# Lagrange-Labs/mapreduce-plonky2

Measured on AMD Instinct MI355X. Metric: leaf proofs/sec (whole node) + NTT GB/s vs HBM peak, 2^20-row table build, 1/2/4/8 GPU, higher is better.
Workload: dtype u64 (Goldilocks field)

## Files before the change

### include/mp2g.h

```cpp
#ifndef MP2G_H
#define MP2G_H
#include <stddef.h>
#include <stdint.h>
#ifdef __cplusplus
extern "C" {
#endif

typedef struct mp2g_ctx mp2g_ctx;
typedef struct mp2g_tree mp2g_tree;
typedef struct mp2g_batch mp2g_batch;

#define MP2G_POSEIDON2 0
#define MP2G_POSEIDON 1

uint64_t mp2g_stat_leaf_permutations(void);
const char* mp2g_last_error(void);
int mp2g_device_count(void);
int mp2g_ctx_create(int device, mp2g_ctx** out);
void mp2g_ctx_destroy(mp2g_ctx* ctx);
int mp2g_ctx_sync(mp2g_ctx* ctx);
int mp2g_ctx_make_current(mp2g_ctx* ctx);
int mp2g_ctx_mem_info(mp2g_ctx* ctx, size_t* free_bytes, size_t* total_bytes);
void* mp2g_ctx_stream(mp2g_ctx* ctx);
int mp2g_ctx_set_stream(mp2g_ctx* ctx, void* stream);
// ... 238 lines not shown
enum mp2g_witness_op_wide {
  MP2G_OP_U32_INTERLEAVE = 48,
  MP2G_OP_UNINTERLEAVE_TO_B32 = 49,
  MP2G_OP_UNINTERLEAVE_TO_U32 = 50,
  MP2G_OP_U256_DIV = 51,
  MP2G_OP_BIGUINT_DIV_REM = 52,
  MP2G_OP_POSEIDON_MDS = 53,
  MP2G_OP_WIDE_END = 54
};
typedef struct mp2g_witness_program mp2g_witness_program;
int mp2g_witness_program_create(const uint64_t* tape, size_t tape_len, uint32_t n_slots, uint32_t log_n, const uint32_t* input_sids,
                                uint32_t n_inputs, const uint64_t* const_slots, uint32_t n_consts, mp2g_witness_program** out);
uint32_t mp2g_witness_program_num_inputs(const mp2g_witness_program* p);
int mp2g_witness_program_set_lookups(mp2g_witness_program* p, const mp2g_lookup* luts, uint32_t n_luts);
uint32_t mp2g_witness_program_num_levels(const mp2g_witness_program* p);
int mp2g_witness_program_set_probe(mp2g_witness_program* p, const uint32_t* probe_sids, uint32_t n_probe);
int mp2g_witness_program_run_dev(mp2g_witness_program* p, mp2g_ctx* ctx, const uint64_t* d_inputs, uint32_t batch, uint64_t* d_wires,
                                 uint64_t* d_probe_out);
int mp2g_witness_program_run(const mp2g_witness_program* p, const uint64_t* inputs, uint32_t batch, uint32_t threads, uint64_t* wires,
                             const uint32_t* probe_sids, uint32_t n_probe, uint64_t* probe_out);
int mp2g_witness_program_run_rows(const mp2g_witness_program* p, const uint64_t* inputs, uint32_t batch, uint32_t threads, uint64_t* rows,
                                  const uint32_t* probe_sids, uint32_t n_probe, uint64_t* probe_out);
int mp2g_wires_from_rows_dev(mp2g_ctx* ctx, const uint64_t* d_rows, uint64_t* d_wires, uint32_t log_n, uint32_t num_wires, uint32_t batch);
void mp2g_witness_program_free(mp2g_witness_program* p);

typedef struct mp2g_chain mp2g_chain;
typedef struct { uint32_t job; uint32_t offset; uint32_t n_words; uint32_t pad_; const uint64_t* d_src; } mp2g_chain_patch;
int mp2g_chain_create(mp2g_ctx* ctx, uint32_t n_steps, mp2g_prover* const* provers, mp2g_witness_program* const* programs,
                      const mp2g_fri_params* params, const uint64_t* const* d_circuit_digests, uint32_t capacity, mp2g_chain** out);
int mp2g_chain_run(mp2g_chain* chain, const uint64_t* inputs, uint32_t batch, const mp2g_chain_patch* patches, uint32_t n_patches,
                   uint64_t* caps, uint64_t* openings, uint64_t* proof, uint64_t* public_inputs);
int mp2g_chain_step_buffers(const mp2g_chain* chain, uint32_t step, uint64_t** d_wires, uint64_t** d_probe, uint64_t** d_caps,
                            uint64_t** d_openings, uint64_t** d_proof);
int mp2g_chain_device_proof(const mp2g_chain* chain, uint32_t b, const uint64_t* d_parts[4], uint32_t n_words[4]);
void mp2g_chain_free(mp2g_chain* chain);

typedef struct mp2g_forest mp2g_forest;
typedef struct {
  uint32_t n_inputs;
  uint32_t n_children;
  uint32_t child_offset[4];
  uint32_t n_const;
} mp2g_forest_circuit;
int mp2g_forest_create(uint32_t n_workers, mp2g_ctx* const* ctxs, uint32_t n_circuits, const mp2g_forest_circuit* circuits,
                       mp2g_chain* const* chains, uint32_t slot_words, uint32_t pool_slots, mp2g_forest** out);
int mp2g_forest_add_nodes(mp2g_forest* f, uint32_t circuit, uint32_t count, const uint64_t* ids, const uint64_t* child_ids ,
                          const uint64_t* consts , const uint8_t* keep );
int mp2g_forest_group_units(const uint32_t* item_sizes, uint32_t n_items, uint32_t n_workers, uint32_t group_nodes,
                            uint32_t* unit_first_item, uint32_t* n_units);
int mp2g_forest_prove(mp2g_forest* f, const uint64_t* unit_nodes, const uint32_t* unit_offsets , uint32_t n_units);
struct mp2g_update_plan;
int mp2g_forest_prove_plan(mp2g_forest* f, struct mp2g_update_plan* plan, uint32_t group_nodes, uint32_t n_satellites, uint32_t satellite_shift,
                           uint32_t* waves, uint32_t* items_per_wave, uint32_t max_waves);
int mp2g_forest_proof(mp2g_forest* f, uint64_t id, uint64_t* words, uint32_t* n_words);
int mp2g_forest_device_proof(mp2g_forest* f, uint64_t id, const uint64_t** d_words, uint32_t* n_words);
int mp2g_forest_release(mp2g_forest* f, uint64_t id);
int mp2g_forest_verify(mp2g_forest* f, mp2g_verifier* v, const uint64_t* ids, uint32_t n_ids, uint32_t* status);
uint64_t mp2g_forest_proved(const mp2g_forest* f);
uint32_t mp2g_forest_free_slots(mp2g_forest* f);
void mp2g_forest_free(mp2g_forest* f);

typedef struct mp2g_update_tree mp2g_update_tree;
typedef struct mp2g_update_plan mp2g_update_plan;
int mp2g_update_tree_from_paths(const uint64_t* keys, const uint32_t* path_lens, uint32_t n_paths, int64_t epoch,
                                mp2g_update_tree** out);
int mp2g_update_tree_from_map(const uint64_t* keys, const uint64_t* left, const uint64_t* right, const uint8_t* has_left,
                              const uint8_t* has_right, uint32_t n, uint64_t root, int64_t epoch, mp2g_update_tree** out);
int mp2g_update_tree_extend_with_path(mp2g_update_tree* t, const uint64_t* path, uint32_t len);
uint32_t mp2g_update_tree_size(const mp2g_update_tree* t);
int64_t mp2g_update_tree_epoch(const mp2g_update_tree* t);
int mp2g_update_tree_contains_key(const mp2g_update_tree* t, uint64_t k);
int mp2g_update_tree_nodes(const mp2g_update_tree* t, uint64_t* keys, int32_t* parents, uint8_t* is_path_end);
int mp2g_update_tree_subtree_size(const mp2g_update_tree* t, uint64_t k, uint32_t* out);
void mp2g_update_tree_free(mp2g_update_tree* t);
int mp2g_update_plan_create(mp2g_update_tree* t, uint32_t subtree_size, mp2g_update_plan** out);
#define MP2G_PLAN_FINISHED 0
#define MP2G_PLAN_READY 1
#define MP2G_PLAN_NOT_YET 2
int mp2g_update_plan_next(mp2g_update_plan* p, uint64_t* k, int* is_path_end, mp2g_update_tree** subtree);
int mp2g_update_plan_done(mp2g_update_plan* p, uint64_t k);
int mp2g_update_plan_completed(const mp2g_update_plan* p);
void mp2g_update_plan_free(mp2g_update_plan* p);

#ifdef __cplusplus
}
#endif
#endif
```

### mapreduce-plonky2_amd/__init__.py

```python
import ctypes
import time
import os
import weakref

import numpy as np

_HERE = os.path.dirname(os.path.abspath(__file__))
LIB_PATH = os.environ.get("MP2G_LIB", os.path.join(_HERE, "libmp2gpu.so"))
HEADER_PATH = os.path.join(os.path.dirname(_HERE), "include", "mp2g.h")

P = 0xFFFFFFFF00000001
MULT_GEN = 14293326489335486720
POSEIDON2, POSEIDON = 0, 1

_u64p = ctypes.POINTER(ctypes.c_uint64)
_u32p = ctypes.POINTER(ctypes.c_uint32)
_lib = None


class Mp2gError(RuntimeError):
    pass


def load():
# ... 658 lines not shown
    def free(self):
        if self.h and self.ctx.h:
            load().mp2g_chain_free(self.h)
        self.h = None

    def __del__(self):
        try:
            self.free()
        except Exception:
            pass


class ForestCircuit(ctypes.Structure):
    _fields_ = [("n_inputs", ctypes.c_uint32), ("n_children", ctypes.c_uint32), ("child_offset", ctypes.c_uint32 * 4), ("n_const", ctypes.c_uint32)]


class Forest:

    def __init__(self, ctxs, descriptors, chains, slot_words, pool_slots):
        self.ctxs, self.chains = list(ctxs), [list(row) for row in chains]
        nw, nc = len(ctxs), len(descriptors)
        d = (ForestCircuit * nc)()
        for i, (n_in, offs, n_const) in enumerate(descriptors):
            d[i].n_inputs, d[i].n_children, d[i].n_const = int(n_in), len(offs), int(n_const)
            for k, o in enumerate(offs):
                d[i].child_offset[k] = int(o)
        cx = (ctypes.c_void_p * nw)(*[c.h for c in ctxs])
        ch = (ctypes.c_void_p * (nw * nc))(*[(self.chains[w][c].h if self.chains[w][c] is not None else None) for w in range(nw) for c in range(nc)])
        self.h = ctypes.c_void_p()
        _ck(load().mp2g_forest_create(nw, cx, nc, d, ch, int(slot_words), int(pool_slots), ctypes.byref(self.h)))
        for c in self.ctxs:
            c._adopt(self)
        self.n_const = [int(x[2]) for x in descriptors]
        self.n_children = [len(x[1]) for x in descriptors]

    def add_nodes(self, circuit, ids, child_ids, consts, keep=None):
        ids = _arr(ids)
        n = ids.size
        kids = _arr(child_ids).reshape(n, self.n_children[circuit]) if self.n_children[circuit] else None
        cs = _arr(consts).reshape(n, self.n_const[circuit])
        kp = np.ascontiguousarray(keep, dtype=np.uint8) if keep is not None else None
        _ck(load().mp2g_forest_add_nodes(self.h, int(circuit), int(n), _p(ids), _p(kids) if kids is not None else None, _p(cs), _p(kp) if kp is not None else None))

    def prove(self, units):
        flat = _arr([i for u in units for i in u])
        offs = _arr(np.cumsum([0] + [len(u) for u in units]), np.uint32)
        _ck(load().mp2g_forest_prove(self.h, _p(flat), _p(offs), len(units)))

    def prove_plan(self, plan, group_nodes, n_satellites=0, satellite_shift=40):
        waves, per = ctypes.c_uint32(), (ctypes.c_uint32 * 64)()
        _ck(load().mp2g_forest_prove_plan(self.h, plan.h, int(group_nodes), int(n_satellites), int(satellite_shift), ctypes.byref(waves), per, 64))
        return [int(per[i]) for i in range(min(64, waves.value))]

    def proof_words(self, node_id):
        n = ctypes.c_uint32()
        _ck(load().mp2g_forest_proof(self.h, ctypes.c_uint64(int(node_id)), None, ctypes.byref(n)))
        out = np.empty(n.value, dtype=np.uint64)
        _ck(load().mp2g_forest_proof(self.h, ctypes.c_uint64(int(node_id)), _p(out), ctypes.byref(n)))
        return out

    def device_proof(self, node_id):
        ptr, n = ctypes.c_void_p(), ctypes.c_uint32()
        _ck(load().mp2g_forest_device_proof(self.h, ctypes.c_uint64(int(node_id)), ctypes.byref(ptr), ctypes.byref(n)))
        return int(ptr.value), int(n.value)

    def verify(self, ids, verifier):
        ids = _arr(ids)
        status = np.full(ids.size, 0xFFFFFFFF, dtype=np.uint32)
        _ck(load().mp2g_forest_verify(self.h, getattr(verifier, "v", verifier).h, _p(ids), int(ids.size), _p(status)))
        return status

    def release(self, node_id):
        _ck(load().mp2g_forest_release(self.h, ctypes.c_uint64(int(node_id))))

    @property
    def proved(self):
        load().mp2g_forest_proved.restype = ctypes.c_uint64
        return int(load().mp2g_forest_proved(self.h))

    def free(self):
        if self.h and all(c.h for c in self.ctxs):
            load().mp2g_forest_free(self.h)
        self.h = None

    def __del__(self):
        try:
            self.free()
        except Exception:
            pass


def map_to_curve_batch(ctx, inputs, variant=POSEIDON2, weierstrass=False):
    a = _arr(inputs)
    count, in_len = a.shape
    w = np.empty((count, 5), dtype=np.uint64)
    wei = np.empty((count, 11), dtype=np.uint64) if weierstrass else None
    _ck(load().mp2g_map_to_curve_batch(ctx.h, variant, _p(a), in_len, count, _p(w), _p(wei) if weierstrass else None))
    return (w, wei) if weierstrass else w


def swu_batch(ctx, u, weierstrass=False):
    a = _arr(u).reshape(-1, 5)
    count = a.shape[0]
    w = np.empty((count, 5), dtype=np.uint64)
    wei = np.empty((count, 11), dtype=np.uint64) if weierstrass else None
    _ck(load().mp2g_swu_batch(ctx.h, _p(a), count, _p(w), _p(wei) if weierstrass else None))
# ... 189 lines not shown
```

### mapreduce-plonky2_amd/csrc/forest.hip

```cpp
#include <algorithm>
#include <atomic>
#include <chrono>
#include <condition_variable>
#include <cstdlib>
#include <cstring>
#include <deque>
#include <exception>
#include <memory>
#include <mutex>
#include <new>
#include <string>
#include <thread>
#include <unordered_map>
#include <vector>
#include "chain.h"
#include "verifier.h"

using namespace mp2g;
extern "C" const char* mp2g_last_error(void);

namespace {
constexpr uint32_t MAX_CHILDREN = 4;
struct Node {
  uint64_t id = 0;
  uint32_t circuit = 0;
  uint32_t n_children = 0;
  uint64_t child[MAX_CHILDREN] = {0, 0, 0, 0};
  size_t consts = 0;
  int32_t slot = -1;
  uint32_t proof_words = 0;
  bool keep = false;
  bool proved = false;
  uint32_t queued_by = 0;
};
struct Circuit {
  mp2g_forest_circuit d{};
  std::vector<u64> consts;
};
struct Copy { const u64* src; u64* dst; uint32_t n; uint32_t pad; };
__global__ void __launch_bounds__(256) forest_copy_kernel(const Copy* jobs) {
  const Copy c = jobs[blockIdx.x];
  for (uint32_t i = threadIdx.x; i < c.n; i += 256) c.dst[i] = c.src[i];
}
}

struct mp2g_forest {
  uint32_t n_workers = 0, n_circuits = 0, slot_words = 0, pool_slots = 0;
  std::vector<mp2g_ctx*> ctxs;
  std::vector<mp2g_chain*> chains;
  std::vector<Circuit> circuits;
  std::unordered_map<uint64_t, uint32_t> index;
  std::vector<Node> nodes;
  DevBuf pool;
  std::vector<int32_t> free_slots;
  std::mutex mu;
  std::condition_variable slots_back;
  uint32_t active = 0, waiting = 0;
  std::atomic<uint64_t> proved{0};
  bool pipelined = true;
  static constexpr uint32_t RING = 3;
  struct Slot { Copy* h_jobs = nullptr; Copy* d_jobs = nullptr; uint32_t* h_flags = nullptr; hipEvent_t done = nullptr; };
  struct Worker { Slot ring[RING]; uint32_t cap_jobs = 0; uint32_t seq = 0; };
  std::vector<Worker> workers;
  ~mp2g_forest() {
    for (auto& w : workers)
      for (auto& r : w.ring) {
        if (r.h_jobs) (void)hipHostFree(r.h_jobs);
        if (r.d_jobs) (void)hipFree(r.d_jobs);
        if (r.h_flags) (void)hipHostFree(r.h_flags);
        if (r.done) (void)hipEventDestroy(r.done);
      }
  }
};

namespace {
struct BatchCtx {
  const Copy* d_jobs; uint32_t n_between, n_after;
};
int hook_copy(const Copy* d_jobs, uint32_t count, hipStream_t s) {
  if (!count) return 0;
  hipLaunchKernelGGL(forest_copy_kernel, dim3(count), dim3(256), 0, s, d_jobs);
  hipError_t e = hipGetLastError();
  return e == hipSuccess ? 0 : fail("forest copy kernel: %s", hipGetErrorString(e));
}
int hook_between(void* u, mp2g_chain*, hipStream_t s) { auto* b = (BatchCtx*)u; return hook_copy(b->d_jobs, b->n_between, s); }
int hook_after(void* u, mp2g_chain*, hipStream_t s) { auto* b = (BatchCtx*)u; return hook_copy(b->d_jobs + b->n_between, b->n_after, s); }

struct InFlight {
  uint32_t ring = 0, B = 0, out_words = 0;
  mp2g_chain* ch = nullptr;
  std::vector<uint32_t> nodes;
  std::vector<int32_t> slots;
};

int prove_unit_body(mp2g_forest* f, uint32_t w, const uint64_t* ids, uint32_t count, std::deque<InFlight>& flight);
int prove_unit(mp2g_forest* f, uint32_t w, const uint64_t* ids, uint32_t count) {
  std::deque<InFlight> flight;
  try {
    return prove_unit_body(f, w, ids, count, flight);
  } catch (...) {
    (void)hipStreamSynchronize(f->ctxs[w]->stream);
    {
      std::lock_guard<std::mutex> g(f->mu);
      for (InFlight& b : flight) {
        for (uint32_t i : b.nodes) { Node& n = f->nodes[i]; n.proved = false; n.queued_by = 0; n.slot = -1; n.proof_words = 0; }
        for (int32_t sl : b.slots) f->free_slots.push_back(sl);
      }
    }
    f->slots_back.notify_all();
    return fail("forest: out of memory (or another exception) inside a unit of worker %u: its queued batches were rolled back", w);
  }
}
// ... 136 lines not shown
            src += end - at;
            at = end;
            if (k < C.d.n_children) {
              Node* ch_node = nullptr;
              {
                std::lock_guard<std::mutex> g(f->mu);
                ch_node = &f->nodes[f->index[n.child[k]]];
                if (!(ch_node->proved || ch_node->queued_by == w + 1) || ch_node->slot < 0) return fail("forest: child %llu of node %llu is not proved (or was released)", (unsigned long long)n.child[k], (unsigned long long)n.id);
              }
              if (at + ch_node->proof_words > C.d.n_inputs) return fail("forest: circuit %u: a child proof runs past the inputs", c);
              R.h_jobs[nb++] = Copy{f->pool.p + (size_t)ch_node->slot * f->slot_words, s0.in.p + (size_t)j * s0.n_in + at, ch_node->proof_words, 0};
              at += ch_node->proof_words;
            }
          }
          if (at != C.d.n_inputs || src != C.consts.data() + n.consts + C.d.n_const)
            return fail("forest: circuit %u: the node's constant words and its children's proofs do not add up to the circuit's %u inputs", c, C.d.n_inputs);
        }
        return 0;
        }();
        if (arc) { give_back(); UNIT_FAIL(arc); }
        const uint32_t n_between = nb;
        for (uint32_t j = 0; j < B; j++) {
          u64* slot = f->pool.p + (size_t)slots[j] * f->slot_words;
          for (uint32_t k = 0; k < 4; k++) R.h_jobs[nb++] = Copy{L.part(k, j), slot + L.parts.off[k], L.parts.n[k], 0};
        }
        {
          hipError_t e = hipMemcpyAsync(R.d_jobs, R.h_jobs, (size_t)nb * sizeof(Copy), hipMemcpyHostToDevice, stream);
          if (e != hipSuccess) { give_back(); UNIT_FAIL(fail("forest: copy jobs upload: %s", hipGetErrorString(e))); }
        }
        memset(R.h_flags, 0, (size_t)ch->n_steps * ch->cap * sizeof(uint32_t));
        BatchCtx bc{R.d_jobs, n_between, nb - n_between};
        ChainHooks hooks{&bc, hook_between, hook_after};
        int rc = chain_enqueue(ch, B, which, &hooks, R.h_flags);
        if (!rc) { hipError_t e = hipEventRecord(R.done, stream); if (e != hipSuccess) rc = fail("forest: event record: %s", hipGetErrorString(e)); }
        if (rc) { std::string msg = mp2g_last_error(); (void)hipStreamSynchronize(stream); give_back(); roll_back(); return fail("%s", msg.c_str()); }
        InFlight fl;
        fl.ring = ring; fl.B = B; fl.out_words = out_words; fl.ch = ch; fl.slots = slots;
        fl.nodes.assign(todo.begin() + lo, todo.begin() + lo + B);
        {
          std::lock_guard<std::mutex> g(f->mu);
          for (uint32_t j = 0; j < B; j++) {
            Node& n = f->nodes[todo[lo + j]];
            n.slot = slots[j]; n.proof_words = out_words; n.queued_by = w + 1;
          }
        }
        flight.push_back(std::move(fl));
      }
    }
  }
  while (!flight.empty()) UNIT_FAIL(confirm_oldest());
#undef UNIT_FAIL
  return 0;
}
}


extern "C" {
int mp2g_forest_create(uint32_t n_workers, mp2g_ctx* const* ctxs, uint32_t n_circuits, const mp2g_forest_circuit* circuits,
                       mp2g_chain* const* chains, uint32_t slot_words, uint32_t pool_slots, mp2g_forest** out) {
  NEED(out && ctxs && circuits && chains && n_workers >= 1 && n_circuits >= 1 && slot_words >= 1 && pool_slots >= 1, "workers / circuits / chains / pool");
  try {
    std::unique_ptr<mp2g_forest> f(new mp2g_forest);
    f->n_workers = n_workers; f->n_circuits = n_circuits; f->slot_words = slot_words; f->pool_slots = pool_slots;
    f->ctxs.assign(ctxs, ctxs + n_workers);
    f->chains.assign(chains, chains + (size_t)n_workers * n_circuits);
    f->circuits.resize(n_circuits);
    uint32_t max_jobs = 0;
    for (uint32_t c = 0; c < n_circuits; c++) {
      const mp2g_forest_circuit& d = circuits[c];
      NEED(d.n_children <= MAX_CHILDREN && d.n_const <= d.n_inputs, "circuit descriptor");
      f->circuits[c].d = d;
      for (uint32_t w = 0; w < n_workers; w++) {
        mp2g_chain* ch = f->chains[(size_t)w * n_circuits + c];
        if (!ch) continue;
        NEED(ch->steps[0].n_in == d.n_inputs, "a chain's base circuit takes another number of inputs than its descriptor says");
        NEED(ch->ctx == ctxs[w], "a worker's chains live on the worker's context");
        max_jobs = std::max(max_jobs, ch->cap * (d.n_children + 4));
      }
    }
    for (uint32_t w = 0; w < n_workers; w++) NEED(ctxs[w] && ctxs[w]->device == ctxs[0]->device, "one forest = one GPU: every worker's context on the same device");
    CK(hipSetDevice(ctxs[0]->device));
    hipError_t e = f->pool.alloc((size_t)slot_words * pool_slots * sizeof(u64));
    if (e != hipSuccess) return fail("forest pool of %u x %u words: %s", pool_slots, slot_words, hipGetErrorString(e));
    f->free_slots.resize(pool_slots);
    for (uint32_t i = 0; i < pool_slots; i++) f->free_slots[i] = (int32_t)(pool_slots - 1 - i);
    f->workers.resize(n_workers);
    uint32_t max_flags = 1;
    for (mp2g_chain* ch : f->chains) if (ch) max_flags = std::max(max_flags, ch->n_steps * ch->cap);
    for (auto& w : f->workers) {
      w.cap_jobs = std::max(1u, max_jobs);
      for (auto& r : w.ring) {
        CK(hipHostMalloc((void**)&r.h_jobs, (size_t)w.cap_jobs * sizeof(Copy), hipHostMallocDefault));
        CK(hipMalloc((void**)&r.d_jobs, (size_t)w.cap_jobs * sizeof(Copy)));
        CK(hipHostMalloc((void**)&r.h_flags, (size_t)max_flags * sizeof(uint32_t), hipHostMallocDefault));
        CK(hipEventCreateWithFlags(&r.done, hipEventDisableTiming));
      }
    }
    { const char* e = getenv("MP2G_FOREST_SYNC"); f->pipelined = !(e && atoi(e)); }
    *out = f.release();
    return 0;
  } catch (const std::bad_alloc&) { return fail("out of memory"); } catch (...) { return fail("internal error"); }
}

int mp2g_forest_add_nodes(mp2g_forest* f, uint32_t circuit, uint32_t count, const uint64_t* ids, const uint64_t* child_ids, const uint64_t* consts,
                          const uint8_t* keep) {
  NEED(f && circuit < f->n_circuits && (ids || !count), "forest / circuit / ids");
  Circuit& C = f->circuits[circuit];
  NEED((child_ids || !C.d.n_children || !count) && (consts || !C.d.n_const || !count), "children / constant words");
  try {
    {
      std::unordered_map<uint64_t, uint32_t> seen;
      seen.reserve(count);
      for (uint32_t i = 0; i < count; i++)
        if (f->index.count(ids[i]) || !seen.emplace(ids[i], i).second) return fail("forest: node %llu registered twice", (unsigned long long)ids[i]);
    }
    for (uint32_t i = 0; i < count; i++) {
      Node n;
      n.id = ids[i]; n.circuit = circuit; n.n_children = C.d.n_children;
      for (uint32_t k = 0; k < C.d.n_children; k++) n.child[k] = child_ids[(size_t)i * C.d.n_children + k];
      n.consts = C.consts.size();
      n.keep = keep && keep[i];
      C.consts.insert(C.consts.end(), consts + (size_t)i * C.d.n_const, consts + (size_t)(i + 1) * C.d.n_const);
      f->index.emplace(n.id, (uint32_t)f->nodes.size());
      f->nodes.push_back(n);
    }
    return 0;
  } catch (const std::bad_alloc&) { return fail("out of memory"); } catch (...) { return fail("internal error"); }
}

int mp2g_forest_prove(mp2g_forest* f, const uint64_t* unit_nodes, const uint32_t* unit_offsets, uint32_t n_units) {
  NEED(f && (n_units == 0 || (unit_nodes && unit_offsets)), "forest / units");
  if (!n_units) return 0;
  std::atomic<uint32_t> next{0};
  std::atomic<int> failed{0};
  std::mutex err_mu;
  std::string err;
  auto leave = [&]() { { std::lock_guard<std::mutex> g(f->mu); if (f->active) f->active--; } f->slots_back.notify_all(); };
  auto work = [&](uint32_t w) {
    struct Leave { decltype(leave)& fn; ~Leave() { fn(); } } on_exit{leave};
    try {
      for (;;) {
        if (failed.load()) return;
        const uint32_t u = next.fetch_add(1);
        if (u >= n_units) return;
        int rc = prove_unit(f, w, unit_nodes + unit_offsets[u], unit_offsets[u + 1] - unit_offsets[u]);
        if (rc) {
          std::lock_guard<std::mutex> g(err_mu);
          if (!failed.exchange(1)) err = mp2g_last_error();
          return;
        }
      }
    } catch (const std::exception& e) {
      std::lock_guard<std::mutex> g(err_mu);
      if (!failed.exchange(1)) err = std::string("internal error: ") + e.what();
    } catch (...) {
      std::lock_guard<std::mutex> g(err_mu);
      if (!failed.exchange(1)) err = "internal error";
    }
  };
  try {
    const uint32_t n_threads = std::min(f->n_workers, n_units);
    { std::lock_guard<std::mutex> g(f->mu); f->active = n_threads; f->waiting = 0; }
    std::vector<std::thread> ts;
    for (uint32_t w = 1; w < n_threads; w++) ts.emplace_back(work, w);
    work(0);
    for (auto& t : ts) t.join();
  } catch (...) {
    return fail("forest: could not start the worker threads");
  }
  if (failed.load()) return fail("%s", err.c_str());
  return 0;
}

int mp2g_forest_group_units(const uint32_t* item_sizes, uint32_t n_items, uint32_t n_workers, uint32_t group_nodes, uint32_t* unit_first_item,
                            uint32_t* n_units) {
  NEED((item_sizes || !n_items) && unit_first_item && n_units && n_workers >= 1, "items / outputs / workers");
  size_t total = 0;
  for (uint32_t i = 0; i < n_items; i++) total += item_sizes[i];
  const size_t cap = std::max<size_t>(1, std::min<size_t>(group_nodes ? group_nodes : 1, (total + n_workers - 1) / n_workers));
  const size_t floor_nodes = std::max<size_t>(1, (group_nodes ? group_nodes : 1) / 6);
  size_t assigned = 0, in_group = 0;
  auto target_now = [&]() -> size_t {
    return std::min(cap, std::max(floor_nodes, (total - assigned) / (2 * (size_t)n_workers)));
  };
  size_t target = target_now();
  uint32_t nu = 0;
  unit_first_item[0] = 0;
  for (uint32_t i = 0; i < n_items; i++) {
    in_group += item_sizes[i];
    if (in_group >= target) { unit_first_item[++nu] = i + 1; assigned += in_group; in_group = 0; target = target_now(); }
  }
  if (in_group) unit_first_item[++nu] = n_items;
  *n_units = nu;
  return 0;
}

int mp2g_forest_prove_plan(mp2g_forest* f, mp2g_update_plan* plan, uint32_t group_nodes, uint32_t n_satellites, uint32_t satellite_shift,
                           uint32_t* waves, uint32_t* items_per_wave, uint32_t max_waves) {
  NEED(f && plan && satellite_shift < 64 && (!n_satellites || satellite_shift > 0), "forest / plan / satellites");
  try {
    uint32_t n_waves = 0;
    for (;;) {
      std::vector<std::vector<uint64_t>> items;
      std::vector<uint64_t> roots;
      for (;;) {
        uint64_t k = 0;
        int end = 0;
        mp2g_update_tree* sub = nullptr;
        const int st = mp2g_update_plan_next(plan, &k, &end, &sub);
        if (st < 0) return 1;
        if (st != MP2G_PLAN_READY) break;
        if (std::find(roots.begin(), roots.end(), k) != roots.end()) { if (sub) mp2g_update_tree_free(sub); continue; }
        std::vector<uint64_t> keys;
        if (sub) {
          keys.resize(mp2g_update_tree_size(sub));
          const int rc = mp2g_update_tree_nodes(sub, keys.data(), nullptr, nullptr);
          mp2g_update_tree_free(sub);
          if (rc) return rc;
        } else {
          keys.push_back(k);
        }
        roots.push_back(k);
        items.push_back(std::move(keys));
      }
      if (items.empty()) break;
      std::vector<uint32_t> sizes(items.size()), first(items.size() + 1);
      for (size_t i = 0; i < items.size(); i++) sizes[i] = (uint32_t)items[i].size();
      uint32_t n_units = 0;
      { const int rg = mp2g_forest_group_units(sizes.data(), (uint32_t)sizes.size(), f->n_workers, group_nodes, first.data(), &n_units); if (rg) return rg; }
      std::vector<uint64_t> nodes;
      std::vector<uint32_t> offs{0};
      for (uint32_t u = 0; u < n_units; u++) {
        for (uint32_t i = first[u]; i < first[u + 1]; i++)
          for (uint64_t k : items[i]) {
            for (uint32_t j = 0; j < n_satellites; j++) nodes.push_back(((uint64_t)(j + 1) << satellite_shift) | k);
            nodes.push_back(k);
          }
        offs.push_back((uint32_t)nodes.size());
      }
      const int rc = mp2g_forest_prove(f, nodes.data(), offs.data(), (uint32_t)offs.size() - 1);
      if (rc) return rc;
      for (uint64_t k : roots) {
        const int rd = mp2g_update_plan_done(plan, k);
        if (rd) return rd;
      }
      if (items_per_wave && n_waves < max_waves) items_per_wave[n_waves] = (uint32_t)items.size();
      n_waves++;
    }
    if (!mp2g_update_plan_completed(plan)) return fail("forest: the work plan stalled with items not done");
    if (waves) *waves = n_waves;
    return 0;
  } catch (const std::bad_alloc&) { return fail("out of memory"); } catch (...) { return fail("internal error"); }
}
// ... 13 lines not shown
  }
  *n_words = n;
  if (!words) return 0;
  CK(hipSetDevice(f->ctxs[0]->device));
  CK(hipMemcpy(words, src, (size_t)n * sizeof(u64), hipMemcpyDeviceToHost));
  return 0;
}

int mp2g_forest_device_proof(mp2g_forest* f, uint64_t id, const uint64_t** d_words, uint32_t* n_words) {
  NEED(f && d_words && n_words, "forest / outputs");
  std::lock_guard<std::mutex> g(f->mu);
  auto it = f->index.find(id);
  if (it == f->index.end()) return fail("forest: unknown node %llu", (unsigned long long)id);
  const Node& nd = f->nodes[it->second];
  if (!nd.proved || nd.slot < 0) return fail("forest: node %llu is not proved (or its proof was released)", (unsigned long long)id);
  *d_words = f->pool.p + (size_t)nd.slot * f->slot_words;
  *n_words = nd.proof_words;
  return 0;
}

int mp2g_forest_release(mp2g_forest* f, uint64_t id) {
  NEED(f, "forest");
  std::lock_guard<std::mutex> g(f->mu);
  auto it = f->index.find(id);
  if (it == f->index.end()) return fail("forest: unknown node %llu", (unsigned long long)id);
  Node& nd = f->nodes[it->second];
  if (nd.slot >= 0) { f->free_slots.push_back(nd.slot); nd.slot = -1; }
  return 0;
}

int mp2g_forest_verify(mp2g_forest* f, mp2g_verifier* v, const uint64_t* ids, uint32_t n_ids, uint32_t* status) {
  NEED(f && v && ids && status && n_ids >= 1, "forest / verifier / ids / status");
  NEED(verifier_ctx(v) && verifier_ctx(v)->device == f->ctxs[0]->device, "the verifier must live on the device of the forest's pool");
  NEED(n_ids <= verifier_capacity(v), "more ids than the verifier's capacity");
  const size_t words = mp2g_verifier_proof_words(v, nullptr);
  std::vector<const u64*> srcs(n_ids);
  {
    std::lock_guard<std::mutex> g(f->mu);
    for (uint32_t i = 0; i < n_ids; i++) {
      auto it = f->index.find(ids[i]);
      if (it == f->index.end()) return fail("forest: unknown node %llu", (unsigned long long)ids[i]);
      const Node& nd = f->nodes[it->second];
      if (!nd.proved || nd.slot < 0) return fail("forest: node %llu is not proved (or its proof was released)", (unsigned long long)ids[i]);
      if (nd.proof_words != words) return fail("forest: node %llu is not a proof of the verifier's circuit (%u words, the verifier takes %zu)",
                                               (unsigned long long)ids[i], nd.proof_words, words);
      srcs[i] = f->pool.p + (size_t)nd.slot * f->slot_words;
    }
  }
  CK(hipSetDevice(f->ctxs[0]->device));
  return verifier_verify_gathered(v, srcs.data(), n_ids, status);
}

uint64_t mp2g_forest_proved(const mp2g_forest* f) { return f ? f->proved.load() : 0; }
uint32_t mp2g_forest_free_slots(mp2g_forest* f) {
  if (!f) return 0;
  std::lock_guard<std::mutex> g(f->mu);
  return (uint32_t)f->free_slots.size();
}

void mp2g_forest_free(mp2g_forest* f) {
  if (!f) return;
  for (mp2g_ctx* c : f->ctxs) if (c) (void)hipStreamSynchronize(c->stream);
  delete f;
}
}
```

### mapreduce-plonky2_amd/csrc/workplan.hip

```cpp
#include <algorithm>
#include <exception>
#include <memory>
#include <new>
#include <set>
#include <unordered_map>
#include <utility>
#include <vector>
#include "ctx.h"

using namespace mp2g;

template <class F> static int guarded(int on_error, F&& f) noexcept {
  try {
    return f();
  } catch (const std::bad_alloc&) {
    fail("out of memory");
  } catch (const std::exception& e) {
    fail("internal error: %s", e.what());
  } catch (...) {
    fail("internal error");
  }
  return on_error;
}

// ... 156 lines not shown
  if (t.nodes.empty()) return MP2G_PLAN_FINISHED;
  if (p->anchors.empty()) return MP2G_PLAN_NOT_YET;
  const uint64_t anchor = p->anchors.back();
  if (p->batch_size == 1) {
    auto it = t.idx.find(anchor);
    if (it == t.idx.end()) { fail("internal error: anchor not in the tree"); return -1; }
    p->anchors.pop_back();
    *k = anchor;
    if (is_path_end) *is_path_end = t.nodes[it->second].is_path_end ? 1 : 0;
    return MP2G_PLAN_READY;
  }
  if (!subtree) { fail("invalid argument: a batched plan needs the subtree out-pointer"); return -1; }
  return guarded(-1, [&]() -> int {
    auto it = t.idx.find(anchor);
    if (it == t.idx.end()) { fail("internal error: anchor not in the tree"); return -1; }
    uint32_t root = it->second;
    while (t.nodes[root].parent >= 0) {
      const uint32_t parent = (uint32_t)t.nodes[root].parent;
      if (t.subtree_size_i(parent) > p->batch_size) break;
      root = parent;
    }
    std::unique_ptr<mp2g_update_tree> sub = t.spin_off(root);
    p->anchors.pop_back();
    *k = t.nodes[root].k;
    if (is_path_end) *is_path_end = t.nodes[root].is_path_end ? 1 : 0;
    *subtree = sub.release();
    return MP2G_PLAN_READY;
  });
}
int mp2g_update_plan_done(mp2g_update_plan* p, uint64_t k) {
  if (!p) return fail("invalid argument: null plan");
  mp2g_update_tree& t = *p->t;
  auto it = t.idx.find(k);
  if (it == t.idx.end()) return fail("key not found");
  const uint32_t i = it->second;
  return guarded(1, [&]() -> int {
    if (i != 0) {
      if (i >= t.nodes.size()) return fail("key not found");
      const uint32_t parent = (uint32_t)t.nodes[i].parent;
      if (t.nodes[parent].children.size() == 1 && t.nodes[parent].children.count(i))
        p->anchors.reserve(p->anchors.size() + 1);
    }
    p->anchors.erase(std::remove(p->anchors.begin(), p->anchors.end(), k), p->anchors.end());
    if (i == 0) {
      t.nodes.clear();
    } else {
      const uint32_t parent = (uint32_t)t.nodes[i].parent;
      t.nodes[parent].children.erase(i);
      if (t.nodes[parent].children.empty()) p->anchors.push_back(t.nodes[parent].k);
    }
    return 0;
  });
}
int mp2g_update_plan_completed(const mp2g_update_plan* p) { return p && p->t->nodes.empty() ? 1 : 0; }
void mp2g_update_plan_free(mp2g_update_plan* p) {
  if (!p) return;
  delete p->t;
  delete p;
}
}
```

### mapreduce-plonky2_amd/table.py

```python
import os
import queue
import threading
import time
from concurrent.futures import ThreadPoolExecutor

import numpy as np

from . import curve_sum_ranges, map_to_curve_batch, row_digests, u256_to_limbs
from . import recursion as R
from . import workplan as W

CELLS_IO = 4 + 11 + 11 + 1 + 1
ROWS_IO = 4 + 11 + 11 + 8 + 8 + 1
NEUTRAL_FIELDS = [0] * 10 + [1]
CELL_LEN = 1 + 8 + 1


def _u64cat(*parts):
    return np.concatenate([np.asarray(x, dtype=np.uint64).ravel() for x in parts])


def sbbst_root(n):
    return 1 << (n.bit_length() - 1) if n > 0 else 0

# ... 487 lines not shown
            m = len(ka)
            if not m:
                continue
            cols, child_cols = [np.broadcast_to(set_r[None, :], (m, 4))], []
            for side in ((), (None,), (0, 1))[("row_leaf", "row_partial", "row_full").index(n)]:
                kid = np.array([(nodes[int(k)][side] if side is not None else next(x for x in nodes[int(k)] if x is not None)) for k in ka], dtype=np.int64)
                child_cols.append(kid.astype(np.uint64))
                cols.append(np.stack([blocks_r[self.row_name[int(x)]][0] for x in kid]))
                cols.append(np.stack([blocks_r[self.row_name[int(x)]][1] for x in kid]))
            cols += [np.broadcast_to(head_c[None, :], (m, head_c.size)), np.broadcast_to(tail_c[None, :], (m, tail_c.size))]
            cols += [np.full((m, 1), table.col_ids[0], dtype=np.uint64), table.values[ka, 0].astype(np.uint64), np.zeros((m, 1), dtype=np.uint64),
                     np.asarray(wit.unique[ka], dtype=np.uint64), np.stack([np.asarray(wit.row_digest[int(k)], dtype=np.uint64) for k in ka]),
                     np.broadcast_to(neutral[None, :], (m, 11))]
            if n == "row_partial":
                cols.append(np.array([[1 if nodes[int(k)][0] is not None else 0] for k in ka], dtype=np.uint64))
            consts = np.ascontiguousarray(np.concatenate(cols, axis=1))
            child_ids = np.stack(child_cols + [(np.uint64(root_c) << np.uint64(40)) | ka.astype(np.uint64)], axis=1)
            kp = np.array([1 if int(k) in keep else 0 for k in ka], dtype=np.uint8)
            self.forest.add_nodes(self.CIRCUITS.index(n), ka.astype(np.uint64), child_ids, consts, kp)

    def _host_proof(self, words, rows_set, name):
        fp, n_pi = (self.fp_rows, self.npi_rows) if rows_set else (self.fp_cells, self.npi_cells)
        cw, no = int(fp.cap_words), int(fp.n_openings)
        caps = np.zeros((4, cw), dtype=np.uint64)
        caps[0] = np.asarray((self.p.rows if rows_set else self.p.cells).vds[name][0], dtype=np.uint64).ravel()
        caps[1:4] = words[n_pi:n_pi + 3 * cw].reshape(3, cw)
        at = n_pi + 3 * cw
        return caps, words[at:at + 2 * no].reshape(no, 2).copy(), words[at + 2 * no:].copy(), words[:n_pi].copy()

    def run(self, table, wit, root, nodes, keep=()):
        from . import Forest
        C = table.n_cols
        keep_rows = set(keep)
        for k in list(keep_rows):
            keep_rows.update(c for c in nodes[k] if c is not None)
        keep_rows.add(root)
        if self.forest is not None:
            self.forest.free()
        unit = max(1, min(self.group_rows, -(-table.rows // len(self.provers))))
        per_row = max(2, cells_tree_live_peak(C))
        slots = self.pool_slots or (len(self.provers) * (per_row * unit + 4 * self.batch) + table.rows // max(1, self.subtree_size // 2) + 2 * len(keep_rows) + 256)
        self.forest = Forest([pv.ctx for pv in self.provers], self.desc, self.chains, max(self.pw_cells, self.pw_rows), slots)
        self.register(table, wit, root, nodes, keep_rows)
        ut = W.UpdateTree.from_map(0, root, nodes)
        plan = ut.into_batched_workplan(self.subtree_size) if self.subtree_size > 1 else ut.into_workplan()
        t0 = time.perf_counter()
        stop = self._progress_writer(t0, (C + 1) * table.rows)
        try:
            items = self.forest.prove_plan(plan, self.group_rows, n_satellites=C, satellite_shift=40)
        finally:
            stop()
        self.wave_log = [(n_items, None, None) for n_items in items]
        self.seconds_in_prove = time.perf_counter() - t0
        assert plan.completed()
        plan.free()
        self.n_proofs += self.forest.proved
        self.row_proofs = {k: (self._host_proof(self.forest.proof_words(k), True, self.row_name[k]), self.row_name[k]) for k in keep_rows}
        self.cells_roots = {k: (self._host_proof(self.forest.proof_words(self.cell_id(k, sbbst_root(C))), False, self.cells_root_name), self.cells_root_name) for k in keep_rows}
        return self.row_proofs[root]

    def _progress_writer(self, t0, total):
        path = os.environ.get("MP2G_PROGRESS_FILE")
        if not path:
            return lambda: None
        import threading
        done, forest = threading.Event(), self.forest

        def loop():
            while not done.wait(30.0):
                with open(path, "a") as f:
                    f.write(f"{time.perf_counter() - t0:.1f} s  {forest.proved} / {total} proofs\n")
        th = threading.Thread(target=loop, daemon=True)
        th.start()

        def stop():
            done.set()
            th.join()
            with open(path, "a") as f:
                f.write(f"{time.perf_counter() - t0:.1f} s  {forest.proved} / {total} proofs (plan done)\n")
        return stop

    def free(self):
        if self.forest is not None:
            self.forest.free()
            self.forest = None
```

Before: 921.1.

## Replace wave barriers with dependency-driven unit release in forest plan proving

Walks the whole update plan up front, records each item's parent, and then releases a parent's proving unit as soon as all its children finish, instead of waiting for the whole wave to complete. Satellite (cells) proofs for a parent can also be dispatched early, as soon as its first child completes. Workers pull units from a shared queue under the forest mutex, which is meant to remove idle time at wave boundaries. The old wave path stays available through an environment variable. Adds timeline stamping and a release-order simulation API for diagnostics, at the cost of extra host bookkeeping and lock traffic.

```diff
diff --git a/include/mp2g.h b/include/mp2g.h
--- a/include/mp2g.h
+++ b/include/mp2g.h
@@ -314,6 +314,9 @@
 struct mp2g_update_plan;
 int mp2g_forest_prove_plan(mp2g_forest* f, struct mp2g_update_plan* plan, uint32_t group_nodes, uint32_t n_satellites, uint32_t satellite_shift,
                            uint32_t* waves, uint32_t* items_per_wave, uint32_t max_waves);
+int mp2g_forest_plan_timeline(mp2g_forest* f, double* seconds, uint32_t* proofs, uint32_t max, uint32_t* n);
+int mp2g_forest_release_order(struct mp2g_update_plan* plan, uint32_t n_workers, uint32_t group_nodes, const uint32_t* picks, uint32_t n_picks,
+                              uint64_t* item_roots, uint32_t* handed_after, uint32_t* done_at, uint32_t max_items, uint32_t* n_items);
 int mp2g_forest_proof(mp2g_forest* f, uint64_t id, uint64_t* words, uint32_t* n_words);
 int mp2g_forest_device_proof(mp2g_forest* f, uint64_t id, const uint64_t** d_words, uint32_t* n_words);
 int mp2g_forest_release(mp2g_forest* f, uint64_t id);
@@ -341,6 +344,7 @@
 #define MP2G_PLAN_NOT_YET 2
 int mp2g_update_plan_next(mp2g_update_plan* p, uint64_t* k, int* is_path_end, mp2g_update_tree** subtree);
 int mp2g_update_plan_done(mp2g_update_plan* p, uint64_t k);
+int mp2g_update_plan_parent(const mp2g_update_plan* p, uint64_t k, uint64_t* parent, int* has_parent);
 int mp2g_update_plan_completed(const mp2g_update_plan* p);
 void mp2g_update_plan_free(mp2g_update_plan* p);
 
diff --git a/mapreduce-plonky2_amd/__init__.py b/mapreduce-plonky2_amd/__init__.py
--- a/mapreduce-plonky2_amd/__init__.py
+++ b/mapreduce-plonky2_amd/__init__.py
@@ -734,6 +734,14 @@
         _ck(load().mp2g_forest_prove_plan(self.h, plan.h, int(group_nodes), int(n_satellites), int(satellite_shift), ctypes.byref(waves), per, 64))
         return [int(per[i]) for i in range(min(64, waves.value))]
 
+    def plan_timeline(self):
+        n = ctypes.c_uint32()
+        _ck(load().mp2g_forest_plan_timeline(self.h, None, None, 0, ctypes.byref(n)))
+        sec, proofs = np.zeros(n.value, dtype=np.float64), np.zeros(n.value, dtype=np.uint32)
+        if n.value:
+            _ck(load().mp2g_forest_plan_timeline(self.h, _p(sec), _p(proofs), n.value, ctypes.byref(n)))
+        return sec, proofs
+
     def proof_words(self, node_id):
         n = ctypes.c_uint32()
         _ck(load().mp2g_forest_proof(self.h, ctypes.c_uint64(int(node_id)), None, ctypes.byref(n)))
diff --git a/mapreduce-plonky2_amd/csrc/forest.hip b/mapreduce-plonky2_amd/csrc/forest.hip
--- a/mapreduce-plonky2_amd/csrc/forest.hip
+++ b/mapreduce-plonky2_amd/csrc/forest.hip
@@ -58,6 +58,12 @@
   uint32_t active = 0, waiting = 0;
   std::atomic<uint64_t> proved{0};
   bool pipelined = true;
+  bool wave_barrier = false;
+  std::condition_variable unit_cv;
+  bool timeline_on = false;
+  std::chrono::steady_clock::time_point plan_t0;
+  std::vector<std::pair<double, uint64_t>> timeline;
+  void stamp() { if (timeline_on) timeline.emplace_back(std::chrono::duration<double>(std::chrono::steady_clock::now() - plan_t0).count(), proved.load()); }
   static constexpr uint32_t RING = 3;
   struct Slot { Copy* h_jobs = nullptr; Copy* d_jobs = nullptr; uint32_t* h_flags = nullptr; hipEvent_t done = nullptr; };
   struct Worker { Slot ring[RING]; uint32_t cap_jobs = 0; uint32_t seq = 0; };
@@ -300,6 +306,188 @@
 #undef UNIT_FAIL
   return 0;
 }
+
+struct PlanItem {
+  uint64_t root = 0;
+  std::vector<uint64_t> keys;
+  int32_t parent = -1;
+  uint32_t pending = 0;
+  bool early_out = false;
+};
+struct Release {
+  std::vector<PlanItem> items;
+  std::vector<uint32_t> per_wave;
+  enum : uint32_t { WHOLE = 0, SATELLITES = 1, NODES = 2 };
+  std::vector<std::vector<uint32_t>> units;
+  size_t items_done = 0;
+  bool satellites_early = false;
+
+  int walk(mp2g_update_plan* plan) {
+    std::vector<uint64_t> above;
+    std::vector<int> has_above;
+    for (;;) {
+      const size_t first = items.size();
+      for (;;) {
+        uint64_t k = 0;
+        int end = 0;
+        mp2g_update_tree* sub = nullptr;
+        const int st = mp2g_update_plan_next(plan, &k, &end, &sub);
+        if (st < 0) return 1;
+        if (st != MP2G_PLAN_READY) break;
+        if (std::find_if(items.begin() + first, items.end(), [&](const PlanItem& it) { return it.root == k; }) != items.end()) { if (sub) mp2g_update_tree_free(sub); continue; }
+        PlanItem it;
+        it.root = k;
+        if (sub) {
+          std::unique_ptr<mp2g_update_tree, void (*)(mp2g_update_tree*)> hold(sub, mp2g_update_tree_free);
+          it.keys.resize(mp2g_update_tree_size(sub));
+          const int rc = mp2g_update_tree_nodes(sub, it.keys.data(), nullptr, nullptr);
+          if (rc) return rc;
+        } else {
+          it.keys.push_back(k);
+        }
+        items.push_back(std::move(it));
+      }
+      if (items.size() == first) break;
+      for (size_t i = first; i < items.size(); i++) {
+        uint64_t up = 0;
+        int has = 0;
+        int rc = mp2g_update_plan_parent(plan, items[i].root, &up, &has);
+        if (!rc) rc = mp2g_update_plan_done(plan, items[i].root);
+        if (rc) return rc;
+        above.push_back(up);
+        has_above.push_back(has);
+      }
+      per_wave.push_back((uint32_t)(items.size() - first));
+    }
+    if (!mp2g_update_plan_completed(plan)) return fail("forest: the work plan stalled with items not done");
+    std::unordered_map<uint64_t, uint32_t> owner;
+    for (size_t i = 0; i < items.size(); i++)
+      for (uint64_t k : items[i].keys) owner.emplace(k, (uint32_t)i);
+    for (size_t i = 0; i < items.size(); i++) {
+      if (!has_above[i]) continue;
+      auto o = owner.find(above[i]);
+      if (o == owner.end() || o->second == i) return fail("forest: the work plan handed out item %llu and never the node above it", (unsigned long long)items[i].root);
+      items[i].parent = (int32_t)o->second;
+      items[o->second].pending++;
+    }
+    return 0;
+  }
+  int first_units(uint32_t n_workers, uint32_t group_nodes, uint32_t* n_units) {
+    std::vector<uint32_t> ready, sizes;
+    for (size_t i = 0; i < items.size(); i++)
+      if (!items[i].pending) { ready.push_back((uint32_t)i); sizes.push_back((uint32_t)items[i].keys.size()); }
+    std::vector<uint32_t> first(ready.size() + 1);
+    *n_units = 0;
+    const int rc = mp2g_forest_group_units(sizes.data(), (uint32_t)sizes.size(), n_workers, group_nodes, first.data(), n_units);
+    if (rc) return rc;
+    for (uint32_t u = 0; u < *n_units; u++) {
+      units.emplace_back();
+      for (uint32_t r = first[u]; r < first[u + 1]; r++) units.back().push_back(ready[r] << 2 | WHOLE);
+    }
+    return 0;
+  }
+  int32_t complete(uint32_t u, int32_t* early = nullptr) {
+    std::vector<uint32_t> arrivals, sats;
+    if (early) *early = -1;
+    for (uint32_t e : units[u]) {
+      const uint32_t i = e >> 2;
+      if ((e & 3) == SATELLITES) {
+        if (--items[i].pending == 0) arrivals.push_back(i << 2 | NODES);
+        continue;
+      }
+      items_done++;
+      const int32_t p = items[i].parent;
+      if (p < 0) continue;
+      if (satellites_early && !items[p].early_out) { items[p].early_out = true; items[p].pending++; sats.push_back((uint32_t)p); }
+      if (--items[p].pending == 0) arrivals.push_back((uint32_t)p << 2 | (items[p].early_out ? NODES : WHOLE));
+    }
+    for (auto it = sats.begin(); it != sats.end();)
+      if (items[*it].pending == 1) { items[*it].pending = 0; arrivals.push_back(*it << 2 | WHOLE); it = sats.erase(it); } else ++it;
+    if (!sats.empty() && early) {
+      for (uint32_t& i : sats) i = i << 2 | SATELLITES;
+      units.push_back(std::move(sats));
+      *early = (int32_t)units.size() - 1;
+    }
+    if (arrivals.empty()) return -1;
+    std::sort(arrivals.begin(), arrivals.end());
+    units.push_back(std::move(arrivals));
+    return (int32_t)units.size() - 1;
+  }
+};
+
+int prove_plan_released(mp2g_forest* f, Release& rel, uint32_t group_nodes, uint32_t n_satellites, uint32_t satellite_shift) {
+  uint32_t n_first = 0;
+  rel.satellites_early = n_satellites > 0;
+  { const int rc = rel.first_units(f->n_workers, group_nodes, &n_first); if (rc) return rc; }
+  std::deque<uint32_t> queue;
+  for (uint32_t u = 0; u < n_first; u++) queue.push_back(u);
+  uint32_t in_flight = 0;
+  bool failed = false;
+  std::string err;
+  auto work = [&](uint32_t w) {
+    std::unique_lock<std::mutex> g(f->mu);
+    auto fail_with = [&](const std::string& m) { if (!failed) { failed = true; err = m; } };
+    try {
+      for (;;) {
+        if (failed || rel.items_done == rel.items.size()) break;
+        if (queue.empty()) {
+          if (!in_flight) { fail_with("forest: the work plan stalled with items not done"); break; }
+          f->unit_cv.wait(g);
+          continue;
+        }
+        const uint32_t u = queue.front();
+        queue.pop_front();
+        in_flight++;
+        f->active++;
+        g.unlock();
+        int rc = 0;
+        std::string msg;
+        try {
+          std::vector<uint64_t> ids;
+          for (uint32_t e : rel.units[u])
+            for (uint64_t k : rel.items[e >> 2].keys) {
+              for (uint32_t j = 0; j < n_satellites && (e & 3) != Release::NODES; j++) ids.push_back(((uint64_t)(j + 1) << satellite_shift) | k);
+              if ((e & 3) != Release::SATELLITES) ids.push_back(k);
+            }
+          rc = prove_unit(f, w, ids.data(), (uint32_t)ids.size());
+          if (rc) msg = mp2g_last_error();
+        } catch (const std::bad_alloc&) { rc = 1; msg = "out of memory"; } catch (...) { rc = 1; msg = "internal error"; }
+        g.lock();
+        in_flight--;
+        f->active--;
+        if (rc) {
+          fail_with(msg);
+        } else {
+          f->stamp();
+          int32_t early = -1;
+          const int32_t nu = rel.complete(u, &early);
+          if (early >= 0) queue.push_front((uint32_t)early);
+          if (nu >= 0) queue.push_front((uint32_t)nu);
+        }
+        f->unit_cv.notify_all();
+        f->slots_back.notify_all();
+      }
+    } catch (...) {
+      if (!g.owns_lock()) g.lock();
+      fail_with("out of memory (or another exception) in the forest's unit queue");
+    }
+    f->unit_cv.notify_all();
+    f->slots_back.notify_all();
+  };
+  { std::lock_guard<std::mutex> g(f->mu); f->active = 0; f->waiting = 0; }
+  std::vector<std::thread> ts;
+  try {
+    const uint32_t n_threads = f->n_workers;
+    for (uint32_t w = 1; w < n_threads; w++) ts.emplace_back(work, w);
+  } catch (...) {
+    std::lock_guard<std::mutex> g(f->mu);
+    if (!failed) { failed = true; err = "forest: could not start the worker threads"; }
+  }
+  work(0);
+  for (auto& t : ts) t.join();
+  if (failed) return fail("%s", err.c_str());
+  return 0;
+}
 }
 
 
@@ -345,6 +533,7 @@
       }
     }
     { const char* e = getenv("MP2G_FOREST_SYNC"); f->pipelined = !(e && atoi(e)); }
+    { const char* e = getenv("MP2G_FOREST_WAVES"); f->wave_barrier = e && atoi(e); }
     *out = f.release();
     return 0;
   } catch (const std::bad_alloc&) { return fail("out of memory"); } catch (...) { return fail("internal error"); }
@@ -397,6 +586,7 @@
           if (!failed.exchange(1)) err = mp2g_last_error();
           return;
         }
+        if (f->timeline_on) { std::lock_guard<std::mutex> g(f->mu); f->stamp(); }
       }
     } catch (const std::exception& e) {
       std::lock_guard<std::mutex> g(err_mu);
@@ -447,6 +637,16 @@
                            uint32_t* waves, uint32_t* items_per_wave, uint32_t max_waves) {
   NEED(f && plan && satellite_shift < 64 && (!n_satellites || satellite_shift > 0), "forest / plan / satellites");
   try {
+    { std::lock_guard<std::mutex> g(f->mu); f->timeline.clear(); f->plan_t0 = std::chrono::steady_clock::now(); f->timeline_on = true; }
+    struct Off { mp2g_forest* f; ~Off() { std::lock_guard<std::mutex> g(f->mu); f->timeline_on = false; } } off{f};
+    if (!f->wave_barrier) {
+      Release rel;
+      { const int rc = rel.walk(plan); if (rc) return rc; }
+      if (!rel.items.empty()) { const int rc = prove_plan_released(f, rel, group_nodes, n_satellites, satellite_shift); if (rc) return rc; }
+      for (uint32_t i = 0; items_per_wave && i < rel.per_wave.size() && i < max_waves; i++) items_per_wave[i] = rel.per_wave[i];
+      if (waves) *waves = (uint32_t)rel.per_wave.size();
+      return 0;
+    }
     uint32_t n_waves = 0;
     for (;;) {
       std::vector<std::vector<uint64_t>> items;
@@ -566,6 +766,46 @@
 }
 
 uint64_t mp2g_forest_proved(const mp2g_forest* f) { return f ? f->proved.load() : 0; }
+
+int mp2g_forest_plan_timeline(mp2g_forest* f, double* seconds, uint32_t* proofs, uint32_t max, uint32_t* n) {
+  NEED(f && n && ((seconds && proofs) || !max), "forest / outputs");
+  std::lock_guard<std::mutex> g(f->mu);
+  *n = (uint32_t)f->timeline.size();
+  for (uint32_t i = 0; i < max && i < f->timeline.size(); i++) { seconds[i] = f->timeline[i].first; proofs[i] = (uint32_t)f->timeline[i].second; }
+  return 0;
+}
+
+int mp2g_forest_release_order(mp2g_update_plan* plan, uint32_t n_workers, uint32_t group_nodes, const uint32_t* picks, uint32_t n_picks,
+                              uint64_t* item_roots, uint32_t* handed_after, uint32_t* done_at, uint32_t max_items, uint32_t* n_items) {
+  NEED(plan && n_workers >= 1 && (picks || !n_picks) && n_items && ((item_roots && handed_after && done_at) || !max_items), "plan / workers / picks / outputs");
+  try {
+    Release rel;
+    { const int rc = rel.walk(plan); if (rc) return rc; }
+    *n_items = (uint32_t)rel.items.size();
+    if (rel.items.size() > max_items) return fail("forest: the plan has %zu items, the outputs have room for %u", rel.items.size(), max_items);
+    if (rel.items.empty()) return 0;
+    uint32_t n_first = 0;
+    { const int rc = rel.first_units(n_workers, group_nodes, &n_first); if (rc) return rc; }
+    std::vector<uint32_t> out_units, at(rel.items.size(), 0);
+    uint32_t handed = 0, step = 0;
+    auto hand_out = [&](uint32_t u) {
+      out_units.push_back(u);
+      for (uint32_t e : rel.units[u]) { at[e >> 2] = handed; item_roots[handed] = rel.items[e >> 2].root; handed_after[handed] = step; done_at[handed] = 0; handed++; }
+    };
+    for (uint32_t u = 0; u < n_first; u++) hand_out(u);
+    while (!out_units.empty()) {
+      const size_t j = n_picks ? picks[step % n_picks] % out_units.size() : 0;
+      const uint32_t u = out_units[j];
+      out_units.erase(out_units.begin() + (ptrdiff_t)j);
+      step++;
+      for (uint32_t e : rel.units[u]) done_at[at[e >> 2]] = step;
+      const int32_t nu = rel.complete(u);
+      if (nu >= 0) hand_out((uint32_t)nu);
+    }
+    if (handed != rel.items.size()) return fail("forest: the work plan stalled with items not done");
+    return 0;
+  } catch (const std::bad_alloc&) { return fail("out of memory"); } catch (...) { return fail("internal error"); }
+}
 uint32_t mp2g_forest_free_slots(mp2g_forest* f) {
   if (!f) return 0;
   std::lock_guard<std::mutex> g(f->mu);
diff --git a/mapreduce-plonky2_amd/csrc/workplan.hip b/mapreduce-plonky2_amd/csrc/workplan.hip
--- a/mapreduce-plonky2_amd/csrc/workplan.hip
+++ b/mapreduce-plonky2_amd/csrc/workplan.hip
@@ -232,6 +232,16 @@
     return 0;
   });
 }
+int mp2g_update_plan_parent(const mp2g_update_plan* p, uint64_t k, uint64_t* parent, int* has_parent) {
+  if (!p || !parent || !has_parent) return fail("invalid argument: null pointer");
+  const mp2g_update_tree& t = *p->t;
+  auto it = t.idx.find(k);
+  if (it == t.idx.end() || it->second >= t.nodes.size()) return fail("key not found");
+  const int32_t up = t.nodes[it->second].parent;
+  *has_parent = up >= 0 ? 1 : 0;
+  *parent = up >= 0 ? t.nodes[up].k : 0;
+  return 0;
+}
 int mp2g_update_plan_completed(const mp2g_update_plan* p) { return p && p->t->nodes.empty() ? 1 : 0; }
 void mp2g_update_plan_free(mp2g_update_plan* p) {
   if (!p) return;
diff --git a/mapreduce-plonky2_amd/table.py b/mapreduce-plonky2_amd/table.py
--- a/mapreduce-plonky2_amd/table.py
+++ b/mapreduce-plonky2_amd/table.py
@@ -563,6 +563,12 @@
             stop()
         self.wave_log = [(n_items, None, None) for n_items in items]
         self.seconds_in_prove = time.perf_counter() - t0
+        self.timeline = self.forest.plan_timeline()
+        if os.environ.get("MP2G_TIMELINE_FILE"):
+            import json
+            with open(os.environ["MP2G_TIMELINE_FILE"], "a") as f:
+                f.write(json.dumps({"rows": int(table.rows), "workers": len(self.provers), "seconds_in_prove": self.seconds_in_prove,
+                                    "seconds": [round(float(x), 4) for x in self.timeline[0]], "proofs": [int(x) for x in self.timeline[1]]}) + "\n")
         assert plan.completed()
         plan.free()
         self.n_proofs += self.forest.proved
```

Result: no change. 923.5, median of 3 (+0.3%).
